# imagemagick/ImageMagick

Measured on AMD Instinct MI355X. Metric: Mpixels/sec GaussianBlur σ=10 + Lanczos 4× resize, 8K RGBA; %HBM-roofline, higher is better.
Workload: dtype f16x2 products, f32 accumulate for the colour sums of both passes; the row pass's alpha (the column pass's weights) as u8 digit products on the i8 matrix cores: exact i32 sums, f64 rounding; 1 GPU; 8192x8192 RGBA Q16 BlurImage(radius=0,sigma=10): 79-tap row pass + 79-tap column pass, Quantum-rounded intermediate, edge clamp, alpha-weighted colour channels; one independent image per GPU (BASELINE configs[1]); precision=fast, config=c2

## Files before the change

imagemagick_amd/csrc/convolve_fused_hybrid.hip:

```cpp
#include "blur_exact_common.hpp"
#include <cmath>
#include <cstdlib>
#include <cstdio>
#include <vector>
#include <type_traits>

namespace mh {

static constexpr int alpha_plane_degree(int stride)
{
  int worst=1;
  for (int g=0; g < 4; g++)
    {
      int count[16]={0,0,0,0,0,0,0,0,0,0,0,0,0,0,0,0};
      for (int i=0; i < 16; i++)
        {
          const int base=(g & 1) == 0 ? (i < 4 ? i : (i < 8 ? i+8 : i+12)) : (i < 8 ? i+4 : (i < 12 ? i+8 : i+16));
          const int lane=base+32*(g >> 1);
          const int e=lane & 15,kq=lane >> 4;
          const int slot=((e*stride+16*kq) % 256)/16;
          count[slot]++;
          worst=count[slot] > worst ? count[slot] : worst;
        }
    }
  return worst;
}

static constexpr int alpha_plane_stride(int extent)
{
  int best=(extent+15) & ~15,best_degree=99;
  for (int stride=(extent+15) & ~15; stride <= extent+96; stride+=16)
    if (alpha_plane_degree(stride) < best_degree)
      {
        best_degree=alpha_plane_degree(stride);
        best=stride;
      }
  return best;
}

template<int NC,bool BLEND>
struct HybridGeometry
{
  typedef Fused16Geometry<NC> F;
  static constexpr int COLS=64,GROUP=16;
  static constexpr int NG=2*NC,NR=NG+1;
  static constexpr int NX=(NC+1)/2;
  static constexpr int XS=F::XS;
  static constexpr int STAGE_CHANNELS=BLEND ? 3 : 4;
  static constexpr int STAGE_PLANE=STAGE_CHANNELS*F::CHR;
  static constexpr int ring_bytes=(int) (2*F::RING_PLANE*sizeof(_Float16));
  static constexpr int stage_bytes=(int) (2*STAGE_PLANE*sizeof(_Float16));
  static constexpr int ASTRIDE=alpha_plane_stride(XS);
  static constexpr int alpha_bytes=BLEND ? 2*GROUP*ASTRIDE : 0;
  static constexpr int sum_bytes=BLEND ? (int) (COLS*GROUP*sizeof(float)) : 0;
  static constexpr int OUT_STRIDE=COLS+1;
  static constexpr int out_bytes=(int) (GROUP*OUT_STRIDE*sizeof(uint2));
  static constexpr int DLP=116;
  static constexpr int digit_bytes=BLEND ? 4*kExactDigits*DLP : 0;
  static constexpr size_t lds_bytes=(size_t) ring_bytes+stage_bytes+alpha_bytes+sum_bytes+out_bytes+digit_bytes;
  static_assert(lds_bytes <= 163840,"more than the 160 KiB of a CU");
  static constexpr int GROUPS_PER_ROW=XS/4;
  static constexpr int FETCH_GROUPS=GROUP*GROUPS_PER_ROW;
  static_assert(FETCH_GROUPS <= 1024,"one staging round");
  static_assert((FETCH_GROUPS % 64) == 0,"whole staging waves");
  static_assert((alpha_bytes % 16) == 0,"aligned planes");
};

#ifdef MH_HYBRID_KNOCK
#define MH_HKNOCKED(bit) ((args.threshold & (bit)) != 0)
#else
#define MH_HKNOCKED(bit) false
#endif

#ifdef MH_HYBRID_TRACE
#define MH_HTRACE_MARK(id) \
  do { \
    if (traced && (g >= 64) && (g < 112)) \
      { \
        const unsigned long long now=__builtin_readcyclecounter(); \
        if (lane == 0) \
          args.trace[((((int) blockIdx.x*16+wave)*48)+(g-64))*12+(id)]=now; \
      } \
  } while (0)
#else
#define MH_HTRACE_MARK(id) do { } while (0)
#endif

template<int NC,int MODE>
__global__ __launch_bounds__(1024)
void blur_fused_hybrid_kernel(BlurExactArgs args)
{
  constexpr int PX=MODE == MFMA_PLAIN3 ? 3 : 4;
  constexpr int SAMPLES=MODE == MFMA_PLAIN3 ? MFMA_PLAIN4 : MODE;
  constexpr bool BLEND=SAMPLES == MFMA_BLEND4;
  typedef unsigned __attribute__((aligned(2))) LooseDword;
  auto load_pixel16=[&](const uint16_t *at) -> uint2
  {
    if constexpr (MODE == MFMA_PLAIN3)
      return make_uint2(*reinterpret_cast<const LooseDword *>(at),(unsigned) at[2]);
    else
      return *reinterpret_cast<const uint2 *>(at);
  };
  auto store_pixel16=[&](uint16_t *at,uint2 value)
  {
    if constexpr (MODE == MFMA_PLAIN3)
      {
        *reinterpret_cast<LooseDword *>(at)=value.x;
        at[2]=(uint16_t) value.y;
      }
    else
      *reinterpret_cast<uint2 *>(at)=value;
  };
  typedef HybridGeometry<NC,BLEND> G;
  typedef Fused16Geometry<NC> F;
  extern __shared__ __attribute__((aligned(16))) unsigned char smem_raw[];
  _Float16 *ring_hi=reinterpret_cast<_Float16 *>(smem_raw);
  _Float16 *ring_lo=ring_hi+F::RING_PLANE;
  _Float16 *stage_hi=reinterpret_cast<_Float16 *>(smem_raw+G::ring_bytes);
  _Float16 *stage_lo=stage_hi+G::STAGE_PLANE;
  unsigned char *alpha_plane=smem_raw+G::ring_bytes+G::stage_bytes;
  float *alpha_weight=reinterpret_cast<float *>(alpha_plane+G::alpha_bytes);
  uint2 *out_tile=reinterpret_cast<uint2 *>(alpha_plane+G::alpha_bytes+G::sum_bytes);
  unsigned char *digit_table=alpha_plane+G::alpha_bytes+G::sum_bytes+G::out_bytes;
  const int tid=(int) threadIdx.x,lane=tid & 63;
  const int wave=__builtin_amdgcn_readfirstlane(tid >> 6);
  const int n=lane & 15,kq=lane >> 4;
  const int K=args.ntaps;
  const int W=args.columns,H=args.rows;

  const int items=args.strips*args.segments;
  const int item=((int) blockIdx.x & 7)*args.items_per_xcd+((int) blockIdx.x >> 3);
  if (item >= items)
    return;
#ifdef MH_HYBRID_TRACE
  const bool traced=(args.trace != nullptr) && (blockIdx.x < 4);
#endif
  const int segment=item/args.strips,strip=item-segment*args.strips;
  const int x0=G::COLS*strip;
  const int block_begin=segment*args.blocks_per_segment;
  const int block_end=block_begin+args.blocks_per_segment < args.blocks ?
    block_begin+args.blocks_per_segment : args.blocks;
  const int nblocks=block_end-block_begin;
  const int out_begin=G::GROUP*block_begin;
  const int in0=out_begin-args.shift;
  const int xin0=x0-args.shift;
  const int ngroups=nblocks+G::NG-1;

  const bool alpha_wave=BLEND && (wave >= 12);
  const int alpha_tile=wave & 3;
  const int alpha_entry=n*G::ASTRIDE+16*alpha_tile+16*kq;
  const int digit_copy=(3-n) & 3;
  const int digit_entry=digit_copy*(kExactDigits*G::DLP)+16*kq+15-n-digit_copy;

  constexpr int NOPERANDS=!BLEND ? 2*NC : (2*NC > (G::NX == 2 ? 6 : 5) ? 2*NC : (G::NX == 2 ? 6 : 5));
  intx4 operand[NOPERANDS];
  uint2 raw[4];
  auto toeplitz_hi=[&](int c) { return __builtin_bit_cast(half8,operand[c]); };
  auto toeplitz_lo=[&](int c) { return __builtin_bit_cast(half8,operand[NC+c]); };
  {
    float *tap_lds=reinterpret_cast<float *>(stage_hi);
    for (int j=tid; j < K; j+=1024)
      tap_lds[j]=args.taps[j];
    if constexpr (BLEND)
      for (int at=tid; at < G::digit_bytes; at+=1024)
        {
          const int copy=at/(kExactDigits*G::DLP),rest=at-copy*(kExactDigits*G::DLP);
          const int j=rest/G::DLP,v=rest-j*G::DLP+copy-15;
          digit_table[at]=(unsigned char) (((v >= 0) && (v < K)) ? args.digits[j*kExactDigitPitch+v] : (signed char) 0);
        }
    __syncthreads();
#pragma unroll
    for (int i=0; i < NOPERANDS; i++)
      operand[i]=intx4{0,0,0,0};
#pragma unroll
    for (int i=0; i < 4; i++)
      raw[i]=make_uint2(0u,0u);
    if (alpha_wave)
      {
        if constexpr (BLEND)
          {
#pragma unroll
            for (int j=0; j < kExactDigits; j++)
              {
                const unsigned *window=reinterpret_cast<const unsigned *>(digit_table+digit_entry+j*G::DLP);
                operand[j]=intx4{(int) window[0],(int) window[1],(int) window[2],(int) window[3]};
              }
            if constexpr (G::NX == 2)
              {
#pragma unroll
                for (int j=0; j < kExactDigits; j++)
                  {
                    const unsigned *window=reinterpret_cast<const unsigned *>(digit_table+digit_entry+64-8*kq+j*G::DLP);
                    if (j < 2)
                      {
                        operand[NOPERANDS-1][2*j]=(int) window[0];
                        operand[NOPERANDS-1][2*j+1]=(int) window[1];
                      }
                    else
                      raw[j-2]=make_uint2(window[0],window[1]);
                  }
              }
          }
      }
    else
      {
#pragma unroll
        for (int c=0; c < NC; c++)
          {
            half8 t_hi,t_lo;
#pragma unroll
            for (int i=0; i < 8; i++)
              {
                int j=32*c+8*kq+i-n;
                const bool inside=(j >= 0) && (j < K);
                j=inside ? j : 0;
                const float tap=inside ? args.tap_scale*tap_lds[j] : 0.0f;
                _Float16 h,l;
                split_f16(tap,h,l);
                t_hi[i]=h;
                t_lo[i]=l;
              }
            operand[c]=__builtin_bit_cast(intx4,t_hi);
            operand[NC+c]=__builtin_bit_cast(intx4,t_lo);
          }
      }
    __syncthreads();
  }

  const bool stager=tid < G::FETCH_GROUPS;
  auto fetch=[&](int g,int srow,int sxg)
  {
    if (stager)
      {
        int y=in0+G::GROUP*(MH_HKNOCKED(256) ? 0 : g)+srow;
        y=y < 0 ? 0 : (y > H-1 ? H-1 : y);
        const int xs=xin0+4*sxg;
        if ((MODE == MFMA_PLAIN3) && (xs >= 0) && (xs+3 <= W-1))
          {
            const uint16_t *at=args.src+pixel_index(y,W,xs)*3;
            const LooseDword *words=reinterpret_cast<const LooseDword *>(at);
            const uint2 a=make_uint2(words[0],words[1]),b=make_uint2(words[2],words[3]),c=make_uint2(words[4],words[5]);
            raw[0]=make_uint2(a.x,a.y & 0xffffu);
            raw[1]=make_uint2((a.y >> 16) | (b.x << 16),b.x >> 16);
            raw[2]=make_uint2(b.y,c.x & 0xffffu);
            raw[3]=make_uint2((c.x >> 16) | (c.y << 16),c.y >> 16);
          }
        else if ((MODE != MFMA_PLAIN3) && (xs >= 0) && (xs+3 <= W-1))
          {
            typedef unsigned LooseQuad __attribute__((ext_vector_type(4),aligned(8)));
            const LooseQuad *at=reinterpret_cast<const LooseQuad *>(args.src+pixel_index(y,W,xs)*4);
            const LooseQuad a=at[0],b=at[1];
            raw[0]=make_uint2(a[0],a[1]);
            raw[1]=make_uint2(a[2],a[3]);
            raw[2]=make_uint2(b[0],b[1]);
            raw[3]=make_uint2(b[2],b[3]);
          }
        else
          {
            int edge=xs;
            asm volatile("" : "+v"(edge));
#pragma unroll
            for (int i=0; i < 4; i++)
              {
                int x=edge+i;
                x=x < 0 ? 0 : (x > W-1 ? W-1 : x);
                raw[i]=load_pixel16(args.src+pixel_index(y,W,x)*PX);
              }
          }
      }
  };
  auto stage_group=[&](int srow,int sxg)
  {
    if (stager)
      {
        f32x2 v[4][2];
        if (MH_HKNOCKED(32))
          quantum_to_samples<MFMA_PLAIN4>(raw,v);
        else
          quantum_to_samples<SAMPLES>(raw,v);
        unsigned char *to=smem_raw+G::ring_bytes+2*(srow*F::SR+4*sxg);
        constexpr int STAGED=MODE == MFMA_PLAIN3 ? 3 : G::STAGE_CHANNELS;
#pragma unroll
        for (int c=0; c < STAGED; c++)
          {
            uint2 hi,lo;
            split_f16_pair(v[c][0],hi.x,lo.x);
            split_f16_pair(v[c][1],hi.y,lo.y);
            *reinterpret_cast<uint2 *>(to+2*c*F::CHR)=hi;
            *reinterpret_cast<uint2 *>(to+2*(G::STAGE_PLANE+c*F::CHR))=lo;
          }
        if constexpr (BLEND)
          if (!MH_HKNOCKED(16))
          {
            const unsigned hy01=__builtin_amdgcn_perm(raw[1].y,raw[0].y,0x07030602u),hy23=__builtin_amdgcn_perm(raw[3].y,raw[2].y,0x07030602u);
            unsigned char *line=smem_raw+G::ring_bytes+G::stage_bytes+srow*G::ASTRIDE+4*sxg;
            *reinterpret_cast<unsigned *>(line)=__builtin_amdgcn_perm(hy23,hy01,0x05040100u) ^ 0x80808080u;
            *reinterpret_cast<unsigned *>(line+G::GROUP*G::ASTRIDE)=__builtin_amdgcn_perm(hy23,hy01,0x07060302u) ^ 0x80808080u;
          }
      }
  };

  static_assert(alpha_plane_degree(2*F::SR) == 1,"the row operands' reads are conflict-free");
  const int rc=wave >> 2,ot=wave & 3;
  const bool row_wave=!(BLEND || (MODE == MFMA_PLAIN3)) || (wave < 12);
  const int row_entry=rc*F::CHR+n*F::SR+16*ot+8*kq;
  constexpr int TILE_WAVES=16-G::FETCH_GROUPS/64-(BLEND ? 4 : 0);
  static_assert(TILE_WAVES >= 1,"somebody runs the column pass");
  constexpr int CT=3;
  constexpr int SPILLED=16 > CT*TILE_WAVES ? 16-CT*TILE_WAVES : 0;
  static_assert(SPILLED <= 4*CT,"four staging waves take the rest");
  const int tile_wave=wave-G::FETCH_GROUPS/64;
  int ctiles=0,ctile0=0;
  if ((tile_wave >= 0) && (tile_wave < TILE_WAVES))
    {
      if constexpr (SPILLED == 0)
        {
          ctiles=16/TILE_WAVES+(tile_wave < 16 % TILE_WAVES ? 1 : 0);
          ctile0=tile_wave*(16/TILE_WAVES)+(tile_wave < 16 % TILE_WAVES ? tile_wave : 16 % TILE_WAVES);
        }
      else
        {
          ctiles=CT;
          ctile0=CT*tile_wave;
        }
    }
  else if ((SPILLED > 0) && (wave < 4))
    {
      ctiles=SPILLED/4+(wave < SPILLED % 4 ? 1 : 0);
      ctile0=CT*TILE_WAVES+wave*(SPILLED/4)+(wave < SPILLED % 4 ? wave : SPILLED % 4);
    }
  constexpr int GROUP_STRIDE=2*F::OB;
  const int col_entry16=(n & 3)*F::CHC+(4*ctile0+(n >> 2))*8+(kq & 1)*F::OB;
  const int ring_entry16=rc*F::CHC+(kq >> 1)*F::OB+(16*ot+n)*8+4*(kq & 1);
  const int ring_alpha16=3*F::CHC+(kq >> 1)*F::OB+(16*alpha_tile+n)*8+4*(kq & 1);
  auto weight_slot=[&](int tile) { return (16*tile+n)*G::GROUP+4*(kq ^ ((n >> 2) & 3)); };
  int ring_group=0;
  unsigned recomputed=0u;

  floatx4 sums_row={0.0f,0.0f,0.0f,0.0f};
  intx4 plane_low={0,0,0,0},plane_high={0,0,0,0};
  long plane_low2=0,plane_high2=0;
  auto store_row=[&](int block,int lane)
  {
    if ((block >= 0) && (block < nblocks))
      {
        const uint2 result=out_tile[wave*G::OUT_STRIDE+lane];
        const int x=x0+lane,y=out_begin+G::GROUP*block+wave;
        if ((x < W) && (y < H) && !MH_HKNOCKED(512))
          store_pixel16(args.dst+pixel_index(y,W,x)*PX,result);
      }
  };
  fetch(0,tid/G::GROUPS_PER_ROW,tid % G::GROUPS_PER_ROW);
  for (int g=0; g <= ngroups+1; g++)
    {
      int opaque_tid=tid;
      asm volatile("" : "+v"(opaque_tid));
      const int srow=opaque_tid/G::GROUPS_PER_ROW,sxg=opaque_tid-srow*G::GROUPS_PER_ROW;
      const int cb=g-G::NG-1;
      const int first=ring_group;
      const int previous=ring_group == 0 ? G::NR-1 : ring_group-1;
      MH_HTRACE_MARK(0);
      if (g < ngroups)
        {
          stage_group(srow,sxg);
          MH_HTRACE_MARK(1);
          if (g+1 < ngroups)
            fetch(g+1,srow,sxg);
        }
      MH_HTRACE_MARK(2);
      if constexpr (BLEND)
        if (alpha_wave && !MH_HKNOCKED(2))
          {
            intx4 tiles[5];
#pragma unroll
            for (int c=0; c < 5; c++)
              tiles[c]=intx4{0,0,0,0};
            if (!MH_HKNOCKED(1))
              {
#pragma unroll
                for (int j=0; j < kExactDigits; j++)
                  tiles[j]=digit_product(plane_high,operand[j],tiles[j]);
#pragma unroll
                for (int j=1; j < kExactDigits; j++)
                  tiles[j-1]=digit_product(plane_low,operand[j],tiles[j-1]);
                if constexpr (G::NX == 2)
                  {
                    auto join=[](unsigned lo,unsigned hi) { return (long) (((unsigned long) hi << 32) | (unsigned long) lo); };
                    const long digit[kExactDigits]={
                      join((unsigned) operand[NOPERANDS-1][0],(unsigned) operand[NOPERANDS-1][1]),
                      join((unsigned) operand[NOPERANDS-1][2],(unsigned) operand[NOPERANDS-1][3]),
                      join(raw[0].x,raw[0].y),join(raw[1].x,raw[1].y),join(raw[2].x,raw[2].y)};
#pragma unroll
                    for (int j=0; j < kExactDigits; j++)
                      tiles[j]=digit_product(plane_high2,digit[j],tiles[j]);
#pragma unroll
                    for (int j=1; j < kExactDigits; j++)
                      tiles[j-1]=digit_product(plane_low2,digit[j],tiles[j-1]);
                  }
              }
            double sums_alpha[4];
            if (!MH_HKNOCKED(8))
              exact_sums(tiles,args.offset,sums_alpha);
            else
              sums_alpha[0]=sums_alpha[1]=sums_alpha[2]=sums_alpha[3]=0.0;
            unsigned q[4];
            const bool doubtful=exact_levels<false>(sums_alpha,args,q);
            const int x=x0+16*alpha_tile+n;
            {
              auto fetch_alpha=[&](int from,int v,unsigned (&level)[4])
              {
                int xx=x0+16*alpha_tile+(from & 15)-args.shift+v;
                xx=xx < 0 ? 0 : (xx > W-1 ? W-1 : xx);
#pragma unroll
                for (int r=0; r < 4; r++)
                  {
                    int yy=in0+G::GROUP*(g-1)+4*(from >> 4)+r;
                    yy=yy < 0 ? 0 : (yy > H-1 ? H-1 : yy);
                    level[r]=(unsigned) args.src[pixel_index(yy,W,xx)*4+3];
                  }
              };
              recomputed+=settle_doubtful_pixels<false,4>(doubtful && (g >= 1) && (g-1 < ngroups) && (x < W),lane,
                args.taps64,K,fetch_alpha,q);
            }
            const float half_level[4]={0.5f*(float) q[0],0.5f*(float) q[1],0.5f*(float) q[2],0.5f*(float) q[3]};
            uint2 hi,lo;
            split_f16_pair(f32x2{half_level[0],half_level[1]},hi.x,lo.x);
            split_f16_pair(f32x2{half_level[2],half_level[3]},hi.y,lo.y);
            const int at=ring_alpha16+previous*GROUP_STRIDE;
            *reinterpret_cast<uint2 *>(ring_hi+at)=hi;
            *reinterpret_cast<uint2 *>(ring_lo+at)=lo;
            floatx4 weight;
#pragma unroll
            for (int r=0; r < 4; r++)
              weight[r]=half_level[r]*args.two_over_scale*__builtin_amdgcn_rcpf((float) (sums_alpha[r]*args.alpha_scale));
            *reinterpret_cast<floatx4 *>(alpha_weight+weight_slot(alpha_tile))=weight;
          }
      MH_HTRACE_MARK(3);
      if ((cb >= 0) && (cb < nblocks))
        {
          int chunk_at[NC];
#pragma unroll
          for (int c=0; c < NC; c++)
            {
              const unsigned wide=(unsigned) (first+2*c+(kq >> 1));
              const unsigned group=wide < wide-(unsigned) G::NR ? wide : wide-(unsigned) G::NR;
              chunk_at[c]=col_entry16+GROUP_STRIDE*(int) group;
            }
          auto column_tiles=[&](auto count,int done)
          {
            constexpr int N=decltype(count)::value;
            floatx4 acc[N];
#pragma unroll
            for (int i=0; i < N; i++)
              acc[i]=floatx4{0.0f,0.0f,0.0f,0.0f};
#pragma unroll
            for (int c=0; c < NC; c++)
              {
                half8 a_hi[N],a_lo[N];
#pragma unroll
                for (int i=0; i < N; i++)
                  {
                    a_hi[i]=*reinterpret_cast<const half8 *>(ring_hi+chunk_at[c]+4*(done+i)*F::SC);
                    a_lo[i]=*reinterpret_cast<const half8 *>(ring_lo+chunk_at[c]+4*(done+i)*F::SC);
                  }
#pragma unroll
                for (int i=0; i < N; i++)
                  acc[i]=__builtin_amdgcn_mfma_f32_16x16x32_f16(a_hi[i],toeplitz_hi(c),acc[i],0,0,0);
#pragma unroll
                for (int i=0; i < N; i++)
                  acc[i]=__builtin_amdgcn_mfma_f32_16x16x32_f16(a_lo[i],toeplitz_hi(c),acc[i],0,0,0);
#pragma unroll
                for (int i=0; i < N; i++)
                  acc[i]=__builtin_amdgcn_mfma_f32_16x16x32_f16(a_hi[i],toeplitz_lo(c),acc[i],0,0,0);
              }
#pragma unroll
            for (int i=0; i < N; i++)
              out_tile[n*G::OUT_STRIDE+4*(ctile0+done+i)+kq]=MH_HKNOCKED(128) ?
                sums_to_quantum<MFMA_PLAIN4>(acc[i][0],acc[i][1],acc[i][2],acc[i][3],args.quantum_unit) :
                sums_to_quantum<SAMPLES>(acc[i][0],acc[i][1],acc[i][2],acc[i][3],args.quantum_unit);
          };
          for (int done=0; done < ctiles; done+=CT)
            {
              const int left=ctiles-done;
              if (left >= CT)
                column_tiles(std::integral_constant<int,CT>{},done);
              else if (left == 2)
                column_tiles(std::integral_constant<int,2>{},done);
              else
                column_tiles(std::integral_constant<int,1>{},done);
            }
        }
      MH_HTRACE_MARK(4);
      __syncthreads();
      MH_HTRACE_MARK(5);
      {
        floatx4 weight={1.0f,1.0f,1.0f,1.0f};
        if constexpr (BLEND)
          if (row_wave && !MH_HKNOCKED(4))
            weight=*reinterpret_cast<const floatx4 *>(alpha_weight+weight_slot(ot));
        if constexpr (BLEND)
          if (alpha_wave)
            {
              plane_low=*reinterpret_cast<const intx4 *>(alpha_plane+alpha_entry);
              plane_high=*reinterpret_cast<const intx4 *>(alpha_plane+G::GROUP*G::ASTRIDE+alpha_entry);
              if constexpr (G::NX == 2)
                {
                  const int at=alpha_entry+64-8*kq;
                  plane_low2=*reinterpret_cast<const long *>(alpha_plane+at);
                  plane_high2=*reinterpret_cast<const long *>(alpha_plane+G::GROUP*G::ASTRIDE+at);
                }
            }
        MH_HTRACE_MARK(6);
        if (row_wave)
          {
            floatx4 acc={0.0f,0.0f,0.0f,0.0f};
#pragma unroll
            for (int c=0; c < NC; c++)
              {
                const half8 a_hi=*reinterpret_cast<const half8 *>(stage_hi+row_entry+32*c);
                const half8 a_lo=*reinterpret_cast<const half8 *>(stage_lo+row_entry+32*c);
                acc=__builtin_amdgcn_mfma_f32_16x16x32_f16(a_hi,toeplitz_hi(c),acc,0,0,0);
                acc=__builtin_amdgcn_mfma_f32_16x16x32_f16(a_lo,toeplitz_hi(c),acc,0,0,0);
                acc=__builtin_amdgcn_mfma_f32_16x16x32_f16(a_hi,toeplitz_lo(c),acc,0,0,0);
              }
            float v[4];
            if (BLEND && !MH_HKNOCKED(64))
              {
#pragma unroll
                for (int r=0; r < 4; r++)
                  v[r]=__builtin_fmaxf(sums_row[r]*weight[r],0.0f);
              }
            else
              {
                const float back=0.5f*args.two_over_scale;
#pragma unroll
                for (int r=0; r < 4; r++)
                  v[r]=sums_row[r]*back;
              }
            uint2 hi,lo;
            split_f16_pair(f32x2{v[0],v[1]},hi.x,lo.x);
            split_f16_pair(f32x2{v[2],v[3]},hi.y,lo.y);
            const int at=ring_entry16+previous*GROUP_STRIDE;
            *reinterpret_cast<uint2 *>(ring_hi+at)=hi;
            *reinterpret_cast<uint2 *>(ring_lo+at)=lo;
            asm volatile("s_nop 7\n\ts_nop 7" : "+v"(acc));
            sums_row=acc;
          }
        store_row(cb,opaque_tid & 63);
      }
      MH_HTRACE_MARK(7);
      __syncthreads();
      MH_HTRACE_MARK(8);
      ring_group=ring_group+1 == G::NR ? 0 : ring_group+1;
    }
  if ((args.recomputed != nullptr) && (recomputed != 0u) && (lane == 0))
    atomicAdd(args.recomputed,(unsigned long long) recomputed);
}

template<int NC,int MODE>
static MhStatus launch_hybrid_typed(const View &src,BlurExactArgs &args)
{
  constexpr bool BLEND=MODE == MFMA_BLEND4;
  typedef HybridGeometry<NC,BLEND> G;
  args.strips=(args.columns+G::COLS-1)/G::COLS;
  args.blocks=(args.rows+G::GROUP-1)/G::GROUP;
  const int cus=compute_units(src.device);
  const int max_segments=args.blocks/16 > 1 ? args.blocks/16 : 1;
  int segments=(cus+args.strips-1)/args.strips;
  segments=segments < 1 ? 1 : (segments > max_segments ? max_segments : segments);
  const int forced_segments=(int) option_long("MAGICKHIP_FUSED_SEGMENTS",0);
  if (forced_segments > 0)
    segments=forced_segments > args.blocks ? args.blocks : forced_segments;
  args.blocks_per_segment=(args.blocks+segments-1)/segments;
  args.segments=(args.blocks+args.blocks_per_segment-1)/args.blocks_per_segment;
  const int items=args.strips*args.segments;
  args.items_per_xcd=(items+7)/8;
  const size_t lds=G::lds_bytes;
  static bool attribute_set[64]={};
  const int slot=src.device >= 0 && src.device < 64 ? src.device : 0;
  if (!attribute_set[slot])
    {
      MH_HIP(hipFuncSetAttribute(reinterpret_cast<const void *>(&blur_fused_hybrid_kernel<NC,MODE>),
        hipFuncAttributeMaxDynamicSharedMemorySize,(int) lds));
      attribute_set[slot]=true;
    }
#ifdef MH_HYBRID_TRACE
  const char *trace_path=option("MAGICKHIP_HYBRID_TRACE");
  const size_t trace_bytes=4u*16u*48u*12u*sizeof(unsigned long long);
  if (trace_path != nullptr)
    {
      MH_HIP(hipMalloc(reinterpret_cast<void **>(&args.trace),trace_bytes));
      MH_HIP(hipMemsetAsync(args.trace,0,trace_bytes,src.stream));
    }
#endif
  {
    ProfileScope prof("blur_fused_hybrid",src.stream);
    hipLaunchKernelGGL((blur_fused_hybrid_kernel<NC,MODE>),dim3((unsigned) (8*args.items_per_xcd)),dim3(1024),lds,
      src.stream,args);
    MH_HIP(hipGetLastError());
  }
#ifdef MH_HYBRID_TRACE
  if (args.trace != nullptr)
    {
      std::vector<unsigned long long> host(trace_bytes/sizeof(unsigned long long));
      MH_HIP(hipMemcpyAsync(host.data(),args.trace,trace_bytes,hipMemcpyDeviceToHost,src.stream));
      MH_HIP(hipStreamSynchronize(src.stream));
      MH_HIP(hipFree(args.trace));
      if (FILE *f=fopen(trace_path,"wb"))
        {
          fwrite(host.data(),1,trace_bytes,f);
          fclose(f);
        }
      args.trace=nullptr;
    }
#endif
  return MH_OK;
}

template<int NC>
static MhStatus launch_hybrid_modes(const View &src,BlurExactArgs &args,bool blend)
{
  if (src.channels == 3)
    return launch_hybrid_typed<NC,MFMA_PLAIN3>(src,args);
  return blend ? launch_hybrid_typed<NC,MFMA_BLEND4>(src,args) : launch_hybrid_typed<NC,MFMA_PLAIN4>(src,args);
}

MhStatus launch_blur_fused_hybrid(const View &src,const View &dst,const double *taps,int ntaps,int shift,
  bool blend,bool *handled)
{
  *handled=false;
  if ((src.quantum != MH_QUANTUM_U16) || (dst.quantum != MH_QUANTUM_U16) ||
      ((src.channels != 4) && ((src.channels != 3) || blend)) ||
      (dst.channels != src.channels) || (src.columns != dst.columns) || (src.rows != dst.rows) || (ntaps < 2))
    return MH_OK;
  if ((src.columns >= (1u << 24)) || (src.rows >= (1u << 24)) ||
      ((unsigned long long) src.columns*src.rows >= (1ull << 32)))
    return MH_OK;
  if (ntaps > 81)
    return MH_OK;
  const ExactTapPlan plan=plan_exact_taps(taps,ntaps);
  if (!plan.ok)
    return MH_OK;
  if (!f16_taps_resolved(taps,ntaps))
    return MH_OK;
  ExactDeviceTaps device;
  MH_TRY(upload_exact_taps(src,taps,ntaps,plan,&device));
  BlurExactArgs args;
  args.tap_scale=f16_tap_scale(taps,ntaps);
  args.two_over_scale=2.0f/args.tap_scale;
  args.quantum_unit=(float) (2.0/((double) args.tap_scale*65535.0));
  args.src=static_cast<const uint16_t *>(src.pixels);
  args.dst=static_cast<uint16_t *>(dst.pixels);
  args.columns=(int) src.columns;
  args.rows=(int) src.rows;
  args.ntaps=ntaps;
  args.shift=shift;
  args.taps64=device.taps64;
  args.taps=device.taps;
  args.digits=device.digits;
  args.offset=plan.offset_plain;
  args.alpha_scale=plan.alpha_scale;
  args.colour_window=plan.colour_window;
  args.alpha_half_window=0.5-plan.alpha_window_plain;
  args.alpha_floor=plan.alpha_floor;
  args.gain=0.0f;
  args.threshold=(int) option_long("MAGICKHIP_HYBRID_KNOCK",0);
  args.recomputed=exact_recomputed_counter(src.device);
  args.give_up=nullptr;
  args.trace=nullptr;
  *handled=true;
  const int nc=(ntaps+15+31)/32;
  if (nc == 1)
    return launch_hybrid_modes<1>(src,args,blend);
  if (nc == 2)
    return launch_hybrid_modes<2>(src,args,blend);
  if (nc == 3)
    return launch_hybrid_modes<3>(src,args,blend);
  *handled=false;
  return MH_OK;
}

}
```

Measured before the change: 132,100 Mpixels/s.

## Use buffer-resource loads/stores for frames under 4 GiB and precompute staging addresses

Adds a non-WIDE kernel variant that reads the source and writes the destination through AMD buffer resources with 32-bit byte offsets and 24-bit multiplies, replacing 64-bit flat address arithmetic. Per-thread staging offsets, the ring byte offsets and the role predicates are hoisted out of the group loop, and ring indexing now works in byte offsets with a branch-free half step. Frames of 4 GiB or more, or runs with an environment override, fall back to the original flat-pointer path. The aim is to cut VALU and SGPR address overhead in the fetch and store paths. It risks changed register pressure and scheduling, and it relies on the buffer range check for correctness.

```diff
diff --git a/imagemagick_amd/csrc/convolve_fused_hybrid.hip b/imagemagick_amd/csrc/convolve_fused_hybrid.hip
--- a/imagemagick_amd/csrc/convolve_fused_hybrid.hip
+++ b/imagemagick_amd/csrc/convolve_fused_hybrid.hip
@@ -6,6 +6,9 @@
 #include <type_traits>
 
 namespace mh {
+
+typedef unsigned uintx2 __attribute__((ext_vector_type(2)));
+typedef unsigned uintx4 __attribute__((ext_vector_type(4)));
 
 static constexpr int alpha_plane_degree(int stride)
 {
@@ -86,7 +89,12 @@
 #define MH_HTRACE_MARK(id) do { } while (0)
 #endif
 
-template<int NC,int MODE>
+__device__ __forceinline__ __amdgpu_buffer_rsrc_t frame_resource(const void *base,unsigned bytes)
+{
+  return __builtin_amdgcn_make_buffer_rsrc(const_cast<void *>(base),(short) 0,(int) bytes,0x00020000);
+}
+
+template<int NC,int MODE,bool WIDE>
 __global__ __launch_bounds__(1024)
 void blur_fused_hybrid_kernel(BlurExactArgs args)
 {
@@ -114,8 +122,6 @@
   typedef HybridGeometry<NC,BLEND> G;
   typedef Fused16Geometry<NC> F;
   extern __shared__ __attribute__((aligned(16))) unsigned char smem_raw[];
-  _Float16 *ring_hi=reinterpret_cast<_Float16 *>(smem_raw);
-  _Float16 *ring_lo=ring_hi+F::RING_PLANE;
   _Float16 *stage_hi=reinterpret_cast<_Float16 *>(smem_raw+G::ring_bytes);
   _Float16 *stage_lo=stage_hi+G::STAGE_PLANE;
   unsigned char *alpha_plane=smem_raw+G::ring_bytes+G::stage_bytes;
@@ -228,48 +234,106 @@
   }
 
   const bool stager=tid < G::FETCH_GROUPS;
-  auto fetch=[&](int g,int srow,int sxg)
+  const int stage_row=tid/G::GROUPS_PER_ROW,stage_xs=xin0+4*(tid % G::GROUPS_PER_ROW);
+  const int stage_to=G::ring_bytes+2*(stage_row*F::SR+4*(tid % G::GROUPS_PER_ROW));
+  const int stage_line=G::ring_bytes+G::stage_bytes+stage_row*G::ASTRIDE+4*(tid % G::GROUPS_PER_ROW);
+  const unsigned interior_columns=W >= 4 ? (unsigned) (W-3) : 0u;
+  constexpr int PIXEL_BYTES=2*PX;
+  __amdgpu_buffer_rsrc_t src_frame=frame_resource(args.src,WIDE ? 0u : (unsigned) W*(unsigned) H*(unsigned) PIXEL_BYTES);
+  __amdgpu_buffer_rsrc_t dst_frame=frame_resource(args.dst,WIDE ? 0u : (unsigned) W*(unsigned) H*(unsigned) PIXEL_BYTES);
+  auto load_pixel_at=[&](unsigned offset) -> uint2
+  {
+    if constexpr (MODE == MFMA_PLAIN3)
+      return make_uint2((unsigned) __builtin_amdgcn_raw_buffer_load_b32(src_frame,(int) offset,0,0),
+        (unsigned) __builtin_amdgcn_raw_buffer_load_b16(src_frame,(int) offset+4,0,0));
+    else
+      {
+        const uintx2 pixel=__builtin_amdgcn_raw_buffer_load_b64(src_frame,(int) offset,0,0);
+        return make_uint2(pixel[0],pixel[1]);
+      }
+  };
+  auto fetch=[&](int g)
   {
     if (stager)
       {
-        int y=in0+G::GROUP*(MH_HKNOCKED(256) ? 0 : g)+srow;
+        int y=in0+G::GROUP*(MH_HKNOCKED(256) ? 0 : g)+stage_row;
         y=y < 0 ? 0 : (y > H-1 ? H-1 : y);
-        const int xs=xin0+4*sxg;
-        if ((MODE == MFMA_PLAIN3) && (xs >= 0) && (xs+3 <= W-1))
-          {
-            const uint16_t *at=args.src+pixel_index(y,W,xs)*3;
-            const LooseDword *words=reinterpret_cast<const LooseDword *>(at);
-            const uint2 a=make_uint2(words[0],words[1]),b=make_uint2(words[2],words[3]),c=make_uint2(words[4],words[5]);
-            raw[0]=make_uint2(a.x,a.y & 0xffffu);
-            raw[1]=make_uint2((a.y >> 16) | (b.x << 16),b.x >> 16);
-            raw[2]=make_uint2(b.y,c.x & 0xffffu);
-            raw[3]=make_uint2((c.x >> 16) | (c.y << 16),c.y >> 16);
-          }
-        else if ((MODE != MFMA_PLAIN3) && (xs >= 0) && (xs+3 <= W-1))
-          {
-            typedef unsigned LooseQuad __attribute__((ext_vector_type(4),aligned(8)));
-            const LooseQuad *at=reinterpret_cast<const LooseQuad *>(args.src+pixel_index(y,W,xs)*4);
-            const LooseQuad a=at[0],b=at[1];
-            raw[0]=make_uint2(a[0],a[1]);
-            raw[1]=make_uint2(a[2],a[3]);
-            raw[2]=make_uint2(b[0],b[1]);
-            raw[3]=make_uint2(b[2],b[3]);
+        const int xs=stage_xs;
+        const bool interior=(unsigned) xs < interior_columns;
+        if constexpr (WIDE)
+          {
+            if ((MODE == MFMA_PLAIN3) && interior)
+              {
+                const uint16_t *at=args.src+pixel_index(y,W,xs)*3;
+                const LooseDword *words=reinterpret_cast<const LooseDword *>(at);
+                const uint2 a=make_uint2(words[0],words[1]),b=make_uint2(words[2],words[3]),c=make_uint2(words[4],words[5]);
+                raw[0]=make_uint2(a.x,a.y & 0xffffu);
+                raw[1]=make_uint2((a.y >> 16) | (b.x << 16),b.x >> 16);
+                raw[2]=make_uint2(b.y,c.x & 0xffffu);
+                raw[3]=make_uint2((c.x >> 16) | (c.y << 16),c.y >> 16);
+              }
+            else if ((MODE != MFMA_PLAIN3) && interior)
+              {
+                typedef unsigned LooseQuad __attribute__((ext_vector_type(4),aligned(8)));
+                const LooseQuad *at=reinterpret_cast<const LooseQuad *>(args.src+pixel_index(y,W,xs)*4);
+                const LooseQuad a=at[0],b=at[1];
+                raw[0]=make_uint2(a[0],a[1]);
+                raw[1]=make_uint2(a[2],a[3]);
+                raw[2]=make_uint2(b[0],b[1]);
+                raw[3]=make_uint2(b[2],b[3]);
+              }
+            else
+              {
+                int edge=xs;
+                asm volatile("" : "+v"(edge));
+#pragma unroll
+                for (int i=0; i < 4; i++)
+                  {
+                    int x=edge+i;
+                    x=x < 0 ? 0 : (x > W-1 ? W-1 : x);
+                    raw[i]=load_pixel16(args.src+pixel_index(y,W,x)*PX);
+                  }
+              }
           }
         else
           {
-            int edge=xs;
-            asm volatile("" : "+v"(edge));
-#pragma unroll
-            for (int i=0; i < 4; i++)
-              {
-                int x=edge+i;
-                x=x < 0 ? 0 : (x > W-1 ? W-1 : x);
-                raw[i]=load_pixel16(args.src+pixel_index(y,W,x)*PX);
+            const unsigned row_pixels=__umul24((unsigned) y,(unsigned) W);
+            if ((MODE == MFMA_PLAIN3) && interior)
+              {
+                const int at=(int) ((row_pixels+(unsigned) xs)*(unsigned) PIXEL_BYTES);
+                const uintx4 ab=__builtin_amdgcn_raw_buffer_load_b128(src_frame,at,0,0);
+                const uintx2 c=__builtin_amdgcn_raw_buffer_load_b64(src_frame,at+16,0,0);
+                raw[0]=make_uint2(ab[0],ab[1] & 0xffffu);
+                raw[1]=make_uint2((ab[1] >> 16) | (ab[2] << 16),ab[2] >> 16);
+                raw[2]=make_uint2(ab[3],c[0] & 0xffffu);
+                raw[3]=make_uint2((c[0] >> 16) | (c[1] << 16),c[1] >> 16);
+              }
+            else if ((MODE != MFMA_PLAIN3) && interior)
+              {
+                const int at=(int) ((row_pixels+(unsigned) xs)*(unsigned) PIXEL_BYTES);
+                const uintx4 a=__builtin_amdgcn_raw_buffer_load_b128(src_frame,at,0,0);
+                const uintx4 b=__builtin_amdgcn_raw_buffer_load_b128(src_frame,at+16,0,0);
+                raw[0]=make_uint2(a[0],a[1]);
+                raw[1]=make_uint2(a[2],a[3]);
+                raw[2]=make_uint2(b[0],b[1]);
+                raw[3]=make_uint2(b[2],b[3]);
+              }
+            else
+              {
+                int edge=xs;
+                asm volatile("" : "+v"(edge));
+#pragma unroll
+                for (int i=0; i < 4; i++)
+                  {
+                    int x=edge+i;
+                    x=x < 0 ? 0 : (x > W-1 ? W-1 : x);
+                    raw[i]=load_pixel_at((row_pixels+(unsigned) x)*(unsigned) PIXEL_BYTES);
+                  }
               }
           }
       }
   };
-  auto stage_group=[&](int srow,int sxg)
+  auto stage_group=[&]()
   {
     if (stager)
       {
@@ -278,7 +342,7 @@
           quantum_to_samples<MFMA_PLAIN4>(raw,v);
         else
           quantum_to_samples<SAMPLES>(raw,v);
-        unsigned char *to=smem_raw+G::ring_bytes+2*(srow*F::SR+4*sxg);
+        unsigned char *to=smem_raw+stage_to;
         constexpr int STAGED=MODE == MFMA_PLAIN3 ? 3 : G::STAGE_CHANNELS;
 #pragma unroll
         for (int c=0; c < STAGED; c++)
@@ -293,7 +357,7 @@
           if (!MH_HKNOCKED(16))
           {
             const unsigned hy01=__builtin_amdgcn_perm(raw[1].y,raw[0].y,0x07030602u),hy23=__builtin_amdgcn_perm(raw[3].y,raw[2].y,0x07030602u);
-            unsigned char *line=smem_raw+G::ring_bytes+G::stage_bytes+srow*G::ASTRIDE+4*sxg;
+            unsigned char *line=smem_raw+stage_line;
             *reinterpret_cast<unsigned *>(line)=__builtin_amdgcn_perm(hy23,hy01,0x05040100u) ^ 0x80808080u;
             *reinterpret_cast<unsigned *>(line+G::GROUP*G::ASTRIDE)=__builtin_amdgcn_perm(hy23,hy01,0x07060302u) ^ 0x80808080u;
           }
@@ -302,7 +366,6 @@
 
   static_assert(alpha_plane_degree(2*F::SR) == 1,"the row operands' reads are conflict-free");
   const int rc=wave >> 2,ot=wave & 3;
-  const bool row_wave=!(BLEND || (MODE == MFMA_PLAIN3)) || (wave < 12);
   const int row_entry=rc*F::CHR+n*F::SR+16*ot+8*kq;
   constexpr int TILE_WAVES=16-G::FETCH_GROUPS/64-(BLEND ? 4 : 0);
   static_assert(TILE_WAVES >= 1,"somebody runs the column pass");
@@ -334,42 +397,60 @@
   const int ring_entry16=rc*F::CHC+(kq >> 1)*F::OB+(16*ot+n)*8+4*(kq & 1);
   const int ring_alpha16=3*F::CHC+(kq >> 1)*F::OB+(16*alpha_tile+n)*8+4*(kq & 1);
   auto weight_slot=[&](int tile) { return (16*tile+n)*G::GROUP+4*(kq ^ ((n >> 2) & 3)); };
-  int ring_group=0;
+  constexpr int GROUP_BYTES=2*GROUP_STRIDE;
+  int first_bytes=0,previous_bytes=(G::NR-1)*GROUP_BYTES;
+  int ring_half=kq >> 1;
+  asm volatile("" : "+v"(ring_half));
   unsigned recomputed=0u;
 
   floatx4 sums_row={0.0f,0.0f,0.0f,0.0f};
   intx4 plane_low={0,0,0,0},plane_high={0,0,0,0};
   long plane_low2=0,plane_high2=0;
-  auto store_row=[&](int block,int lane)
+  const int store_from=wave*G::OUT_STRIDE+lane;
+  const bool store_column=x0+lane < W;
+  auto store_row=[&](int block)
   {
     if ((block >= 0) && (block < nblocks))
       {
-        const uint2 result=out_tile[wave*G::OUT_STRIDE+lane];
-        const int x=x0+lane,y=out_begin+G::GROUP*block+wave;
-        if ((x < W) && (y < H) && !MH_HKNOCKED(512))
-          store_pixel16(args.dst+pixel_index(y,W,x)*PX,result);
+        const int y=out_begin+G::GROUP*block+wave;
+        if (store_column && (y < H) && !MH_HKNOCKED(512))
+          {
+            const uint2 result=out_tile[store_from];
+            if constexpr (WIDE)
+              store_pixel16(args.dst+pixel_index(y,W,x0+lane)*PX,result);
+            else
+              {
+                const int row_bytes=(int) (((unsigned) y*(unsigned) W+(unsigned) x0)*(unsigned) PIXEL_BYTES);
+                if constexpr (MODE == MFMA_PLAIN3)
+                  {
+                    __builtin_amdgcn_raw_buffer_store_b32(result.x,dst_frame,lane*PIXEL_BYTES,row_bytes,0);
+                    __builtin_amdgcn_raw_buffer_store_b16((unsigned short) result.y,dst_frame,lane*PIXEL_BYTES+4,row_bytes,0);
+                  }
+                else
+                  __builtin_amdgcn_raw_buffer_store_b64(uintx2{result.x,result.y},dst_frame,lane*PIXEL_BYTES,row_bytes,0);
+              }
+          }
       }
   };
-  fetch(0,tid/G::GROUPS_PER_ROW,tid % G::GROUPS_PER_ROW);
+  fetch(0);
   for (int g=0; g <= ngroups+1; g++)
     {
-      int opaque_tid=tid;
-      asm volatile("" : "+v"(opaque_tid));
-      const int srow=opaque_tid/G::GROUPS_PER_ROW,sxg=opaque_tid-srow*G::GROUPS_PER_ROW;
       const int cb=g-G::NG-1;
-      const int first=ring_group;
-      const int previous=ring_group == 0 ? G::NR-1 : ring_group-1;
+      int role=wave;
+      asm volatile("" : "+s"(role));
+      const bool alpha_now=BLEND && (role >= 12);
+      const bool row_now=!(BLEND || (MODE == MFMA_PLAIN3)) || (role < 12);
       MH_HTRACE_MARK(0);
       if (g < ngroups)
         {
-          stage_group(srow,sxg);
+          stage_group();
           MH_HTRACE_MARK(1);
           if (g+1 < ngroups)
-            fetch(g+1,srow,sxg);
+            fetch(g+1);
         }
       MH_HTRACE_MARK(2);
       if constexpr (BLEND)
-        if (alpha_wave && !MH_HKNOCKED(2))
+        if (alpha_now && !MH_HKNOCKED(2))
           {
             intx4 tiles[5];
 #pragma unroll
@@ -426,9 +507,9 @@
             uint2 hi,lo;
             split_f16_pair(f32x2{half_level[0],half_level[1]},hi.x,lo.x);
             split_f16_pair(f32x2{half_level[2],half_level[3]},hi.y,lo.y);
-            const int at=ring_alpha16+previous*GROUP_STRIDE;
-            *reinterpret_cast<uint2 *>(ring_hi+at)=hi;
-            *reinterpret_cast<uint2 *>(ring_lo+at)=lo;
+            unsigned char *at=smem_raw+(2*ring_alpha16+previous_bytes);
+            *reinterpret_cast<uint2 *>(at)=hi;
+            *reinterpret_cast<uint2 *>(at+2*F::RING_PLANE)=lo;
             floatx4 weight;
 #pragma unroll
             for (int r=0; r < 4; r++)
@@ -442,9 +523,10 @@
 #pragma unroll
           for (int c=0; c < NC; c++)
             {
-              const unsigned wide=(unsigned) (first+2*c+(kq >> 1));
-              const unsigned group=wide < wide-(unsigned) G::NR ? wide : wide-(unsigned) G::NR;
-              chunk_at[c]=col_entry16+GROUP_STRIDE*(int) group;
+              int even=first_bytes+2*c*GROUP_BYTES;
+              even=even >= G::NR*GROUP_BYTES ? even-G::NR*GROUP_BYTES : even;
+              const int step=even == (G::NR-1)*GROUP_BYTES ? -(G::NR-1)*GROUP_BYTES : GROUP_BYTES;
+              chunk_at[c]=__mul24(ring_half,step)+2*col_entry16+even;
             }
           auto column_tiles=[&](auto count,int done)
           {
@@ -460,8 +542,8 @@
 #pragma unroll
                 for (int i=0; i < N; i++)
                   {
-                    a_hi[i]=*reinterpret_cast<const half8 *>(ring_hi+chunk_at[c]+4*(done+i)*F::SC);
-                    a_lo[i]=*reinterpret_cast<const half8 *>(ring_lo+chunk_at[c]+4*(done+i)*F::SC);
+                    a_hi[i]=*reinterpret_cast<const half8 *>(smem_raw+chunk_at[c]+8*(done+i)*F::SC);
+                    a_lo[i]=*reinterpret_cast<const half8 *>(smem_raw+chunk_at[c]+2*F::RING_PLANE+8*(done+i)*F::SC);
                   }
 #pragma unroll
                 for (int i=0; i < N; i++)
@@ -494,12 +576,8 @@
       __syncthreads();
       MH_HTRACE_MARK(5);
       {
-        floatx4 weight={1.0f,1.0f,1.0f,1.0f};
         if constexpr (BLEND)
-          if (row_wave && !MH_HKNOCKED(4))
-            weight=*reinterpret_cast<const floatx4 *>(alpha_weight+weight_slot(ot));
-        if constexpr (BLEND)
-          if (alpha_wave)
+          if (alpha_now)
             {
               plane_low=*reinterpret_cast<const intx4 *>(alpha_plane+alpha_entry);
               plane_high=*reinterpret_cast<const intx4 *>(alpha_plane+G::GROUP*G::ASTRIDE+alpha_entry);
@@ -511,8 +589,12 @@
                 }
             }
         MH_HTRACE_MARK(6);
-        if (row_wave)
-          {
+        if (row_now)
+          {
+            floatx4 weight={1.0f,1.0f,1.0f,1.0f};
+            if constexpr (BLEND)
+              if (!MH_HKNOCKED(4))
+                weight=*reinterpret_cast<const floatx4 *>(alpha_weight+weight_slot(ot));
             floatx4 acc={0.0f,0.0f,0.0f,0.0f};
 #pragma unroll
             for (int c=0; c < NC; c++)
@@ -540,25 +622,26 @@
             uint2 hi,lo;
             split_f16_pair(f32x2{v[0],v[1]},hi.x,lo.x);
             split_f16_pair(f32x2{v[2],v[3]},hi.y,lo.y);
-            const int at=ring_entry16+previous*GROUP_STRIDE;
-            *reinterpret_cast<uint2 *>(ring_hi+at)=hi;
-            *reinterpret_cast<uint2 *>(ring_lo+at)=lo;
+            unsigned char *at=smem_raw+(2*ring_entry16+previous_bytes);
+            *reinterpret_cast<uint2 *>(at)=hi;
+            *reinterpret_cast<uint2 *>(at+2*F::RING_PLANE)=lo;
             asm volatile("s_nop 7\n\ts_nop 7" : "+v"(acc));
             sums_row=acc;
           }
-        store_row(cb,opaque_tid & 63);
+        store_row(cb);
       }
       MH_HTRACE_MARK(7);
       __syncthreads();
       MH_HTRACE_MARK(8);
-      ring_group=ring_group+1 == G::NR ? 0 : ring_group+1;
+      previous_bytes=first_bytes;
+      first_bytes=first_bytes+GROUP_BYTES == G::NR*GROUP_BYTES ? 0 : first_bytes+GROUP_BYTES;
     }
   if ((args.recomputed != nullptr) && (recomputed != 0u) && (lane == 0))
     atomicAdd(args.recomputed,(unsigned long long) recomputed);
 }
 
-template<int NC,int MODE>
-static MhStatus launch_hybrid_typed(const View &src,BlurExactArgs &args)
+template<int NC,int MODE,bool WIDE>
+static MhStatus launch_hybrid_sized(const View &src,BlurExactArgs &args)
 {
   constexpr bool BLEND=MODE == MFMA_BLEND4;
   typedef HybridGeometry<NC,BLEND> G;
@@ -580,7 +663,7 @@
   const int slot=src.device >= 0 && src.device < 64 ? src.device : 0;
   if (!attribute_set[slot])
     {
-      MH_HIP(hipFuncSetAttribute(reinterpret_cast<const void *>(&blur_fused_hybrid_kernel<NC,MODE>),
+      MH_HIP(hipFuncSetAttribute(reinterpret_cast<const void *>(&blur_fused_hybrid_kernel<NC,MODE,WIDE>),
         hipFuncAttributeMaxDynamicSharedMemorySize,(int) lds));
       attribute_set[slot]=true;
     }
@@ -595,7 +678,7 @@
 #endif
   {
     ProfileScope prof("blur_fused_hybrid",src.stream);
-    hipLaunchKernelGGL((blur_fused_hybrid_kernel<NC,MODE>),dim3((unsigned) (8*args.items_per_xcd)),dim3(1024),lds,
+    hipLaunchKernelGGL((blur_fused_hybrid_kernel<NC,MODE,WIDE>),dim3((unsigned) (8*args.items_per_xcd)),dim3(1024),lds,
       src.stream,args);
     MH_HIP(hipGetLastError());
   }
@@ -615,6 +698,15 @@
     }
 #endif
   return MH_OK;
+}
+
+template<int NC,int MODE>
+static MhStatus launch_hybrid_typed(const View &src,BlurExactArgs &args)
+{
+  const unsigned long long bytes=(unsigned long long) src.columns*src.rows*(MODE == MFMA_PLAIN3 ? 6u : 8u);
+  if ((bytes >= (1ull << 32)) || (option_long("MAGICKHIP_HYBRID_WIDE",0) != 0))
+    return launch_hybrid_sized<NC,MODE,true>(src,args);
+  return launch_hybrid_sized<NC,MODE,false>(src,args);
 }
 
 template<int NC>
```

New measurement: 132,900 Mpixels/s, median of 6. Within noise of the previous version (+0.6%).
